# recursiveGecko/Formula-VAD

Measured on AMD Instinct MI355X. Metric: 20ms audio frames/sec end-to-end VAD pipeline, higher is better.
Workload: dtype f32

## Files before the change

formula-vad_amd/binding.py:

```python
import ctypes as C
import os

import numpy as np

_HERE = os.path.dirname(os.path.abspath(__file__))
LIB_PATH = os.environ.get("FVAD_LIB_PATH") or os.path.join(_HERE, "libfvad_hip.so")

c_float_p = C.POINTER(C.c_float)
vp = C.c_void_p
sz = C.c_size_t

FVAD_OK = 0
FVAD_ERR_NO_DEVICE = -101
FVAD_ERR_INVALID_ARGUMENT = -100
FVAD_ERR_OUT_OF_RANGE = -6
FVAD_ERR_NEGATIVE_FREQUENCY = -7
FVAD_ERR_BUFFER_TOO_SMALL = -106
FVAD_ERR_MODEL_FORMAT = -104


class FvadError(RuntimeError):
    def __init__(self, status, where, detail=""):
        self.status = status
        name = lib().fvad_status_name(status).decode()
# ... 808 lines not shown
        try:
            self.close()
        except Exception:
            pass


class VadBatch:

    def __init__(self, n_streams, n_channels=1, sample_rate=48000, fft_size=1024, overrides=None):
        cfg = VadConfig()
        lib().fvad_vad_config_default(C.byref(cfg))
        for k, v in (overrides or {}).items():
            setattr(cfg, k, v)
        self.h = vp()
        check(lib().fvad_vad_batch_create(C.byref(cfg), sample_rate, n_channels, fft_size, n_streams, C.byref(self.h)),
              "fvad_vad_batch_create")
        self.n_streams, self.n_channels = n_streams, n_channels

    def run(self, band, chunk_rms, n_threads=1, chunk_size=24000):
        assert band.dtype == np.float32 and chunk_rms.dtype == np.float32 and band.flags["C_CONTIGUOUS"] and chunk_rms.flags["C_CONTIGUOUS"]
        assert band.shape[0] == chunk_rms.shape[0] == self.n_streams * self.n_channels
        check(lib().fvad_vad_batch_run(self.h, fptr(band), band.shape[1], band.shape[1], fptr(chunk_rms), chunk_rms.shape[1],
                                       chunk_rms.shape[1], chunk_size, n_threads), "fvad_vad_batch_run")
        n = lib().fvad_vad_batch_total_segments(self.h)
        arr = (SpeechSegment * max(n, 1))()
        offs = (sz * (self.n_streams + 1))()
        check(lib().fvad_vad_batch_segments(self.h, arr, max(n, 1), offs), "fvad_vad_batch_segments")
        flat = [(a.sample_from, a.sample_to, a.avg_channel_vol_ratio, a.vad_met_sec) for a in arr[:n]]
        return [flat[offs[s]:offs[s + 1]] for s in range(self.n_streams)]

    def _segments(self):
        n = lib().fvad_vad_batch_total_segments(self.h)
        arr = (SpeechSegment * max(n, 1))()
        offs = (sz * (self.n_streams + 1))()
        check(lib().fvad_vad_batch_segments(self.h, arr, max(n, 1), offs), "fvad_vad_batch_segments")
        flat = [(a.sample_from, a.sample_to, a.avg_channel_vol_ratio, a.vad_met_sec) for a in arr[:n]]
        return [flat[offs[s]:offs[s + 1]] for s in range(self.n_streams)]

    def run_part(self, band, chunk_rms, first_frame, n_threads=1, chunk_size=24000, want_segments=True):
        assert band.dtype == np.float32 and chunk_rms.dtype == np.float32
        assert (band.shape[1] <= 1 or band.strides[1] == 4) and (chunk_rms.shape[1] <= 1 or chunk_rms.strides[1] == 4)
        assert band.shape[0] == chunk_rms.shape[0] == self.n_streams * self.n_channels
        bp = C.cast(band.ctypes.data, c_float_p)
        rp = C.cast(chunk_rms.ctypes.data, c_float_p)
        check(lib().fvad_vad_batch_run_part(self.h, bp, band.strides[0] // 4, band.shape[1], rp, chunk_rms.strides[0] // 4, chunk_rms.shape[1],
                                            chunk_size, first_frame, n_threads), "fvad_vad_batch_run_part")
        return self._segments() if want_segments else None

    def audit(self, stream):
        a = VadAudit()
        check(lib().fvad_vad_batch_audit(self.h, stream, C.byref(a)), "fvad_vad_batch_audit")
        return a.min_rel_threshold_margin, a.min_abs_ratio_margin, a.n_frames

    def close(self):
        if self.h:
            lib().fvad_vad_batch_destroy(self.h)
            self.h = vp()


def _config_array(configs):
    arr = (VadConfig * len(configs))()
    for i, ov in enumerate(configs):
        lib().fvad_vad_config_default(C.byref(arr[i]))
        for k, v in (ov or {}).items():
            setattr(arr[i], k, v)
    return arr


class VadSweep:

    def __init__(self, n_streams, configs, n_channels=1, sample_rate=48000, fft_size=1024):
        self.h = vp()
        check(lib().fvad_vad_batch_create_sweep(_config_array(configs), len(configs), sample_rate, n_channels, fft_size, n_streams,
                                                C.byref(self.h)), "fvad_vad_batch_create_sweep")
        self._created(n_streams, n_channels, len(configs))

    def _created(self, n_streams, n_channels, n_configs):
        self.n_streams, self.n_channels, self.n_configs = n_streams, n_channels, n_configs
        assert lib().fvad_vad_batch_n_configs(self.h) == self.n_configs
        self.sizes, self.size_of_band = self.frame_sizes()

    def frame_sizes(self):
        n = sz()
        sizes = (sz * self.n_configs)()
        sob = (C.c_uint32 * self.n_configs)()
        check(lib().fvad_vad_batch_frame_sizes(self.h, sizes, self.n_configs, C.byref(n), sob), "fvad_vad_batch_frame_sizes")
        n_bands = sz()
        lib().fvad_vad_batch_bands(self.h, None, 0, C.byref(n_bands), None)
        return [sizes[g] for g in range(n.value)], [sob[j] for j in range(n_bands.value)]

    def bands(self):
        n = sz()
        cap = 2 * self.n_configs
        bins = (C.c_int32 * cap)()
        band_of = (C.c_uint32 * self.n_configs)()
        check(lib().fvad_vad_batch_bands(self.h, bins, self.n_configs, C.byref(n), band_of), "fvad_vad_batch_bands")
        return [(bins[2 * j], bins[2 * j + 1]) for j in range(n.value)], list(band_of)

    def size_blocks(self):
        bins, _ = VadSweep.bands(self)
        out = []
        for g, F in enumerate(self.sizes):
            js = [j for j in range(len(bins)) if self.size_of_band[j] == g]
            out.append((F, js[0], [bins[j] for j in js]))
        return out

# ... 423 lines not shown
```

formula-vad_amd/csrc/host_vad.cpp:

```cpp
#include <algorithm>
#include <atomic>
#include <cmath>
#include <cstdlib>
#include <cstring>
#include <memory>
#include <thread>
#include <vector>

#include "host_vad.h"
#include "vad_avgs.h"
#include "vad_finish.h"
#include "vad_ratio.h"

namespace fvad {

RollingAverage::RollingAverage(size_t count, bool has_initial, double initial_val)
    : data(count ? count : 1, 0.0), len(count)
{
    if (has_initial) {
        std::fill(data.begin(), data.begin() + (long)count, initial_val);
        written_count = count;
        avg();
        if (count) enter_steady();
    }
}

double RollingAverage::avg()
{
    double a = 0.0;
    const double scalar = 1.0 / (double)written_count;
    const double* d = data.data();
    for (size_t i = 0; i < written_count; ++i) a += d[i] * scalar;
    last_avg = a;
    has_last_avg = true;
    return a;
}

double RollingAverage::push(float sample)
{
    if (steady) {
        const size_t w = write_idx;
        data[w] = (double)sample;
        q[w] = data[w] * scalar;
        double acc = (w == 0) ? 0.0 : pref;
        acc += q[w];
        const double new_pref = acc;
        const double* qq = q.data();
        for (size_t i = w + 1; i < len; ++i) acc += qq[i];
        last_avg = acc;
        has_last_avg = true;
        write_idx = (w + 1) % len;
        pref = (write_idx == 0) ? 0.0 : new_pref;
        return acc;
    }
    data[write_idx] = (double)sample;
    write_idx = (write_idx + 1) % len;
    if (written_count < len) written_count += 1;
    const double a = avg();
    if (written_count == len && write_idx == 0) enter_steady();
    return a;
}

void RollingAverage::enter_steady()
{
    scalar = 1.0 / (double)len;
    q.resize(len);
    for (size_t i = 0; i < len; ++i) q[i] = data[i] * scalar;
    pref = 0.0;
    for (size_t i = 0; i < write_idx; ++i) pref += q[i];
    steady = true;
}

void Metadata::push(const MetaResult& v, float weight)
{
    if (v.has_ratio) {
        if (!has_ratio) { has_ratio = true; ratio_sum = 0.0f; ratio_weight = 0.0f; }
        ratio_sum += v.volume_ratio * weight;
        ratio_weight += weight;
    }
    if (v.has_min && (!has_min || v.volume_min < volume_min)) { has_min = true; volume_min = v.volume_min; }
    if (v.has_max && (!has_max || v.volume_max > volume_max)) { has_max = true; volume_max = v.volume_max; }
}

MetaResult Metadata::to_result() const
{
    MetaResult r;
    r.has_min = has_min; r.volume_min = volume_min;
    r.has_max = has_max; r.volume_max = volume_max;
    if (has_ratio) { r.has_ratio = true; r.volume_ratio = ratio_sum / ratio_weight; }
    return r;
}

MetaResult analyse_volume(const float* channel_rms, size_t n_channels)
{
    float vol_min = 1, vol_max = 0;
    for (size_t c = 0; c < n_channels; ++c) {
        const float vol = channel_rms[c];
        if (vol < vol_min) vol_min = vol;
        if (vol > vol_max) vol_max = vol;
    }
    MetaResult r;
    r.has_ratio = r.has_min = r.has_max = true;
    r.volume_ratio = (vol_max == 0) ? 0 : vol_min / vol_max;
    r.volume_min = vol_min;
    r.volume_max = vol_max;
    return r;
}

int vad_machine_cfg(const fvad_vad_config& c, size_t sample_rate, size_t fft_size, VadMachineCfg* out)
{
    const float sample_rate_f = (float)sample_rate;
    const float fft_size_f = (float)fft_size;
    const float eval_per_sec = sample_rate_f / fft_size_f;
    const size_t long_len = std::max<size_t>(1, (size_t)(eval_per_sec * c.long_term_speech_avg_sec));
    const size_t short_len = std::max<size_t>(1, (size_t)(eval_per_sec * c.short_term_speech_avg_sec));
    const size_t ratio_len = (size_t)(eval_per_sec * c.channel_vol_ratio_avg_sec);
    VadMachineCfg& k = *out;
    k.lt_scalar = 1.0 / (double)long_len;
    k.st_scalar = 1.0 / (double)short_len;
    k.cr_scalar = 1.0 / (double)ratio_len;
    k.lt_q_init = c.initial_long_term_avg * k.lt_scalar;
    k.initial = c.initial_long_term_avg;
    k.factor = (double)c.speech_threshold_factor;
    k.ratio_threshold = (double)c.channel_vol_ratio_threshold;
    const double n = (double)long_len;
    k.gamma = n * kU / (1.0 - n * kU);
    k.min_open = (uint64_t)(sample_rate_f * c.min_consecutive_sec_to_open);
    k.max_gap = (uint64_t)(sample_rate_f * c.max_speech_gap_sec);
    k.start_buffer = (uint64_t)(sample_rate_f * 2);
    k.end_buffer = (uint64_t)(sample_rate_f * 2);
    k.input_len_sec = fft_size_f / sample_rate_f;
    k.sample_rate_f = sample_rate_f;
    k.min_vad_duration_sec = c.min_vad_duration_sec;
    k.long_len = (uint32_t)long_len;
    k.short_len = (uint32_t)short_len;
    k.ratio_len = (uint32_t)ratio_len;
    k.has_init = c.has_initial_long_term_avg != 0;
    k.band = 0;
    if (ratio_len == 0 || long_len > 0xFFFFFFFFu || short_len > 0xFFFFFFFFu || ratio_len > 0xFFFFFFFFu) return FVAD_ERR_INVALID_ARGUMENT;
    return FVAD_OK;
}

VadMachine::VadMachine(const fvad_vad_config& c, size_t sample_rate, size_t n_channels_, size_t fft_size)
    : n_channels(n_channels_), long_term(1, false, 0), short_term(1, false, 0), ch_ratio(1, false, 0)
{
    vad_machine_cfg(c, sample_rate, fft_size, &cf);
    long_term = RollingAverage(cf.long_len, cf.has_init != 0, cf.initial);
    short_term = RollingAverage(cf.short_len, false, 0);
    ch_ratio = RollingAverage(cf.ratio_len, false, 0);
    lt_last = long_term.last_avg;
    has_last = long_term.has_last_avg;
    segments.reserve(100);
    const char* eager = getenv("FVAD_VAD_EAGER");
    lt_lazy = !(eager && eager[0] == '1');
}

void VadMachine::long_term_exact()
{
    const double* qq = long_term.q.data();
    double acc = 0.0, abs_sum = 0.0;
    for (size_t i = 0; i < long_term.len; ++i) {
        acc += qq[i];
        abs_sum += std::fabs(qq[i]);
    }
    anchor(acc, abs_sum);
}

void VadMachine::long_term_push(float mv)
{
    RollingAverage& a = long_term;
    if (!a.steady || !lt_lazy) {
        const bool was_steady = a.steady;
        lt_last = a.push(mv);
        has_last = true;
        if (lt_lazy && !was_steady && a.steady) long_term_exact();
        return;
    }
    if (!lt_anchored) long_term_exact();
    const size_t w = a.write_idx;
    const double qn = (double)mv * a.scalar, qo = a.q[w];
    a.data[w] = (double)mv;
    a.q[w] = qn;
    a.write_idx = (w + 1) % a.len;
    if (lazy_update(qn, qo)) long_term_exact();
}

float VadMachine::min_volume(const float* channel_volumes) const
{
    float min_v = 999, max_v = 0;
    for (size_t c = 0; c < n_channels; ++c) {
        const float v = channel_volumes[c];
        if (v < min_v) min_v = v;
        if (v > max_v) max_v = v;
    }
    (void)max_v;
    return min_v;
}

fvad_vad_result VadMachine::run(uint64_t index, const float* channel_volumes, bool has_ratio, float ratio)
{
    const float mv = min_volume(channel_volumes);
    const double st = short_term.push(mv);
    const double cr = ch_ratio.push(has_ratio ? ratio : 0);
    const bool met = decide(cf, st, cr, [&] { long_term_exact(); });
    if (!met) long_term_push(mv);
    return finish_step(cf, index, met, has_ratio, ratio, [&](const fvad_speech_segment& s) { segments.push_back(s); });
}

void deal(size_t n, int n_threads, const std::function<void(size_t)>& fn)
{
    const int nt = (int)std::min<size_t>((size_t)std::max(n_threads, 1), n);
    if (nt <= 1) { for (size_t i = 0; i < n; ++i) fn(i); return; }
    std::vector<std::thread> th;
    std::atomic<size_t> next{0};
    for (int t = 0; t < nt; ++t)
        th.emplace_back([&]() { for (;;) { const size_t i = next.fetch_add(1); if (i >= n) break; fn(i); } });
    for (auto& t : th) t.join();
}

void run_many(VadMachine* const* vads, size_t n_streams, const float* const* band,
              const float* const* ratio, const size_t* n_frames, size_t n_channels,
              const uint64_t* first_index, size_t fft_size, int n_threads)
{
    deal(n_streams, n_threads, [&](size_t s) {
        VadMachine* m = vads[s];
        for (size_t k = 0; k < n_frames[s]; ++k) {
            const float r = ratio[s][k];
            const bool has_ratio = !std::isnan(r);
            m->run(first_index[s] + (uint64_t)k * fft_size, band[s] + k * n_channels, has_ratio, r);
        }
    });
}

}

struct fvad_vad { fvad::VadMachine m; fvad_vad(const fvad_vad_config& c, size_t sr, size_t nc, size_t fs) : m(c, sr, nc, fs) {} };
struct fvad_rolling_average { fvad::RollingAverage ra; fvad_rolling_average(size_t n, bool h, double v) : ra(n, h, v) {} };

extern "C" {

void fvad_vad_config_default(fvad_vad_config* c)
{
    c->speech_min_freq = 500; c->speech_max_freq = 2000;
    c->long_term_speech_avg_sec = 180; c->has_initial_long_term_avg = 1; c->initial_long_term_avg = 0.005;
    c->short_term_speech_avg_sec = 0.2f; c->speech_threshold_factor = 10;
    c->channel_vol_ratio_avg_sec = 0.5f; c->channel_vol_ratio_threshold = 0.5f;
    c->min_consecutive_sec_to_open = 0.2f; c->max_speech_gap_sec = 2; c->min_vad_duration_sec = 0.7f;
}

int fvad_vad_create(const fvad_vad_config* cfg, size_t sample_rate, size_t n_channels, size_t fft_size, fvad_vad** out)
{
    if (!cfg || !out || n_channels == 0 || fft_size == 0 || sample_rate == 0) return FVAD_ERR_INVALID_ARGUMENT;
    fvad::VadMachineCfg k;
    if (const int rc = fvad::vad_machine_cfg(*cfg, sample_rate, fft_size, &k)) return rc;
    *out = new (std::nothrow) fvad_vad(*cfg, sample_rate, n_channels, fft_size);
    return *out ? FVAD_OK : FVAD_ERR_ALLOC_FAILED;
}
void fvad_vad_destroy(fvad_vad* v) { delete v; }

int fvad_vad_run(fvad_vad* v, uint64_t index, const float* channel_volumes, int has_ratio, float volume_ratio, fvad_vad_result* out)
{
    if (!v || !channel_volumes) return FVAD_ERR_INVALID_ARGUMENT;
    const fvad_vad_result r = v->m.run(index, channel_volumes, has_ratio != 0, volume_ratio);
    if (out) *out = r;
    return FVAD_OK;
}
size_t fvad_vad_segment_count(const fvad_vad* v) { return v ? v->m.segments.size() : 0; }
int fvad_vad_segments(const fvad_vad* v, fvad_speech_segment* out, size_t cap, size_t* n)
{
    if (!v || !n) return FVAD_ERR_INVALID_ARGUMENT;
    *n = v->m.segments.size();
    if (cap < *n) return FVAD_ERR_BUFFER_TOO_SMALL;
    if (*n) memcpy(out, v->m.segments.data(), *n * sizeof(fvad_speech_segment));
    return FVAD_OK;
}
int fvad_vad_lazy_stats(const fvad_vad* v, uint64_t* exact_evaluations, uint64_t* lazy_pushes)
{
    if (!v) return FVAD_ERR_INVALID_ARGUMENT;
    if (exact_evaluations) *exact_evaluations = v->m.exact_evals;
    if (lazy_pushes) *lazy_pushes = v->m.lazy_pushes;
    return FVAD_OK;
}

int fvad_vad_audit_get(const fvad_vad* v, fvad_vad_audit* out)
{
    if (!v || !out) return FVAD_ERR_INVALID_ARGUMENT;
    *out = v->m.audit;
    return FVAD_OK;
}

int fvad_vad_run_many(fvad_vad* const* vads, size_t n_streams, const float* const* band, const float* const* ratio,
                      const size_t* n_frames, size_t n_channels, const uint64_t* first_index, size_t fft_size, int n_threads)
{
    if (!vads || !band || !ratio || !n_frames || !first_index) return FVAD_ERR_INVALID_ARGUMENT;
    std::vector<fvad::VadMachine*> ms(n_streams);
    for (size_t i = 0; i < n_streams; ++i) {
        if (!vads[i] || vads[i]->m.n_channels != n_channels) return FVAD_ERR_CHANNEL_COUNT_MISMATCH;
        ms[i] = &vads[i]->m;
    }
    fvad::run_many(ms.data(), n_streams, band, ratio, n_frames, n_channels, first_index, fft_size, n_threads);
    return FVAD_OK;
}

int fvad_ra_create(size_t count, int has_initial, double initial_val, fvad_rolling_average** out)
{
    if (!out || count == 0) return FVAD_ERR_INVALID_ARGUMENT;
    *out = new (std::nothrow) fvad_rolling_average(count, has_initial != 0, initial_val);
    return *out ? FVAD_OK : FVAD_ERR_ALLOC_FAILED;
}
void fvad_ra_destroy(fvad_rolling_average* ra) { delete ra; }
double fvad_ra_push(fvad_rolling_average* ra, float sample) { return ra->ra.push(sample); }
int fvad_ra_last_avg(const fvad_rolling_average* ra, double* out)
{
    if (ra->ra.has_last_avg && out) *out = ra->ra.last_avg;
    return ra->ra.has_last_avg ? 1 : 0;
}

int fvad_vad_batch_create(const fvad_vad_config* cfg, size_t sample_rate, size_t n_channels, size_t fft_size, size_t n_streams,
                          fvad_vad_batch** out)
{
    if (!cfg || !out || n_channels == 0 || fft_size == 0 || sample_rate == 0 || n_streams == 0) return FVAD_ERR_INVALID_ARGUMENT;
    fvad::VadMachineCfg k;
    if (const int rc = fvad::vad_machine_cfg(*cfg, sample_rate, fft_size, &k)) return rc;
    auto* b = new (std::nothrow) fvad_vad_batch();
    if (!b) return FVAD_ERR_ALLOC_FAILED;
    b->cfgs.assign(1, *cfg); b->sample_rate = sample_rate; b->n_channels = n_channels; b->fft_size = fft_size; b->n_streams = n_streams;
    const float bin_width = (float)sample_rate / (float)fft_size;
    b->bins = {(int32_t)roundf(cfg->speech_min_freq / bin_width), (int32_t)roundf(cfg->speech_max_freq / bin_width)};
    b->band_of.assign(1, 0);
    b->sizes.assign(1, fft_size); b->size_of.assign(1, 0); b->size_of_band.assign(1, 0);
    b->segs.resize(n_streams);
    b->audits.resize(n_streams);
    b->exact_evals.assign(n_streams, 0);
    b->lazy_pushes.assign(n_streams, 0);
    if (const int rc = fvad::derive_avg_keys(b)) { delete b; return rc; }
    if (const int rc = fvad::derive_trigger_keys(b)) { delete b; return rc; }
    *out = b;
    return FVAD_OK;
}

static int check_sweep_config(const fvad_vad_config& c, size_t sample_rate, size_t fft_size, int32_t* lo, int32_t* hi)
{
    const float bin_width = (float)sample_rate / (float)fft_size;
    const float nyq = (float)sample_rate / 2;
    if (c.speech_min_freq > nyq || c.speech_max_freq > nyq) return FVAD_ERR_OUT_OF_RANGE;
    if (c.speech_min_freq < 0 || c.speech_max_freq < 0) return FVAD_ERR_NEGATIVE_FREQUENCY;
    *lo = (int32_t)roundf(c.speech_min_freq / bin_width);
    *hi = (int32_t)roundf(c.speech_max_freq / bin_width);
    if (*hi < *lo) return FVAD_ERR_INVALID_ARGUMENT;
    fvad::VadMachineCfg k;
    return fvad::vad_machine_cfg(c, sample_rate, fft_size, &k);
}

static int make_sweep(const fvad_vad_config* cfgs, size_t n_configs, const std::vector<size_t>& sizes, const std::vector<uint32_t>& size_of,
                      size_t sample_rate, size_t n_channels, size_t n_streams, fvad_vad_batch** out)
{
    std::vector<std::vector<int32_t>> bins(sizes.size());
    std::vector<uint32_t> local(n_configs);
    for (size_t c = 0; c < n_configs; ++c) {
        int32_t lo = 0, hi = 0;
        const int rc = check_sweep_config(cfgs[c], sample_rate, sizes[size_of[c]], &lo, &hi);
        if (rc) return rc;
        std::vector<int32_t>& bg = bins[size_of[c]];
        size_t j = 0;
        while (j < bg.size() / 2 && !(bg[2 * j] == lo && bg[2 * j + 1] == hi)) ++j;
        if (j == bg.size() / 2) { bg.push_back(lo); bg.push_back(hi); }
        local[c] = (uint32_t)j;
    }
    auto* b = new (std::nothrow) fvad_vad_batch();
    if (!b) return FVAD_ERR_ALLOC_FAILED;
    std::vector<uint32_t> first(sizes.size());
    for (size_t g = 0; g < sizes.size(); ++g) {
        first[g] = (uint32_t)(b->bins.size() / 2);
        b->bins.insert(b->bins.end(), bins[g].begin(), bins[g].end());
        b->size_of_band.insert(b->size_of_band.end(), bins[g].size() / 2, (uint32_t)g);
    }
    b->band_of.resize(n_configs);
    for (size_t c = 0; c < n_configs; ++c) b->band_of[c] = first[size_of[c]] + local[c];
    b->cfgs.assign(cfgs, cfgs + n_configs); b->sample_rate = sample_rate; b->n_channels = n_channels; b->fft_size = sizes[0];
    b->n_streams = n_streams;
    b->sizes = sizes;
    b->size_of = size_of;
    b->segs.resize(n_streams * n_configs);
    b->audits.resize(n_streams * n_configs);
    b->exact_evals.assign(n_streams * n_configs, 0);
    b->lazy_pushes.assign(n_streams * n_configs, 0);
    if (const int rc = fvad::derive_avg_keys(b)) { delete b; return rc; }
    if (const int rc = fvad::derive_trigger_keys(b)) { delete b; return rc; }
    *out = b;
    return FVAD_OK;
}

int fvad_vad_batch_create_sweep(const fvad_vad_config* cfgs, size_t n_configs, size_t sample_rate, size_t n_channels, size_t fft_size,
                                size_t n_streams, fvad_vad_batch** out)
{
    if (!cfgs || !out || n_configs == 0 || n_channels == 0 || fft_size == 0 || sample_rate == 0 || n_streams == 0) return FVAD_ERR_INVALID_ARGUMENT;
    return make_sweep(cfgs, n_configs, {fft_size}, std::vector<uint32_t>(n_configs, 0), sample_rate, n_channels, n_streams, out);
}

int fvad_vad_batch_create_sweep_sized(const fvad_vad_config* cfgs, const size_t* fft_sizes, size_t n_configs, size_t sample_rate,
                                      size_t n_channels, size_t n_streams, fvad_vad_batch** out)
{
    if (!cfgs || !fft_sizes || !out || n_configs == 0 || n_channels == 0 || sample_rate == 0 || n_streams == 0) return FVAD_ERR_INVALID_ARGUMENT;
    std::vector<size_t> sizes;
    std::vector<uint32_t> size_of(n_configs);
    for (size_t c = 0; c < n_configs; ++c) {
        const size_t F = fft_sizes[c];
        if (F < 4 || F > 16384 || F % 2) return FVAD_ERR_INVALID_ARGUMENT;
        size_t g = 0;
        while (g < sizes.size() && sizes[g] != F) ++g;
        if (g == sizes.size()) sizes.push_back(F);
        size_of[c] = (uint32_t)g;
    }
    return make_sweep(cfgs, n_configs, sizes, size_of, sample_rate, n_channels, n_streams, out);
}

int fvad_vad_batch_frame_sizes(const fvad_vad_batch* b, size_t* sizes, size_t cap, size_t* n_sizes, uint32_t* size_of_band)
{
    if (!b || !n_sizes) return FVAD_ERR_INVALID_ARGUMENT;
    *n_sizes = b->sizes.size();
    if (size_of_band) memcpy(size_of_band, b->size_of_band.data(), b->size_of_band.size() * sizeof(uint32_t));
    if (cap < *n_sizes) return FVAD_ERR_BUFFER_TOO_SMALL;
    if (!sizes) return FVAD_ERR_INVALID_ARGUMENT;
    memcpy(sizes, b->sizes.data(), b->sizes.size() * sizeof(size_t));
    return FVAD_OK;
}

void fvad_vad_batch_destroy(fvad_vad_batch* b) { delete b; }

size_t fvad_vad_batch_n_configs(const fvad_vad_batch* b) { return b ? b->cfgs.size() : 0; }

int fvad_vad_batch_avg_keys(const fvad_vad_batch* b, uint32_t* st_keys, uint32_t* cr_keys, size_t cap, size_t* n_st_keys,
                            size_t* n_cr_keys, uint32_t* st_key, uint32_t* cr_key)
{
    if (!b || !n_st_keys || !n_cr_keys) return FVAD_ERR_INVALID_ARGUMENT;
    *n_st_keys = b->st_keys.size() / 2;
    *n_cr_keys = b->cr_keys.size() / 2;
    if (st_key) memcpy(st_key, b->st_key.data(), b->st_key.size() * sizeof(uint32_t));
    if (cr_key) memcpy(cr_key, b->cr_key.data(), b->cr_key.size() * sizeof(uint32_t));
    if (cap < *n_st_keys || cap < *n_cr_keys) return FVAD_ERR_BUFFER_TOO_SMALL;
    if (!st_keys || !cr_keys) return FVAD_ERR_INVALID_ARGUMENT;
// ... 74 lines not shown

namespace fvad {

int derive_avg_keys(fvad_vad_batch* b)
{
    const size_t NC = b->cfgs.size();
    b->st_keys.clear(); b->cr_keys.clear();
    b->st_key.assign(NC, 0); b->cr_key.assign(NC, 0);
    auto find = [](std::vector<uint32_t>& keys, uint32_t src, uint32_t len) {
        size_t j = 0;
        while (j < keys.size() / 2 && !(keys[2 * j] == src && keys[2 * j + 1] == len)) ++j;
        if (j == keys.size() / 2) { keys.push_back(src); keys.push_back(len); }
        return (uint32_t)j;
    };
    for (size_t c = 0; c < NC; ++c) {
        VadMachineCfg k;
        if (const int rc = vad_machine_cfg(b->cfgs[c], b->sample_rate, b->sizes[b->size_of[c]], &k)) return rc;
        b->st_key[c] = find(b->st_keys, b->band_of[c], k.short_len);
        b->cr_key[c] = find(b->cr_keys, b->size_of[c], k.ratio_len);
    }
    return FVAD_OK;
}

int derive_trigger_keys(fvad_vad_batch* b)
{
    struct Key {
        uint32_t size, band, long_len, short_len, ratio_len;
        int32_t has_init;
        uint64_t initial, factor, ratio_threshold;
        bool operator==(const Key& o) const
        {
            return size == o.size && band == o.band && long_len == o.long_len && short_len == o.short_len && ratio_len == o.ratio_len &&
                   has_init == o.has_init && initial == o.initial && factor == o.factor && ratio_threshold == o.ratio_threshold;
        }
    };
    auto bits = [](double d) { uint64_t u; memcpy(&u, &d, 8); return u; };
    const size_t NC = b->cfgs.size();
    std::vector<Key> keys;
    b->trig_key.assign(NC, 0);
    b->trig_rep.clear();
    for (size_t c = 0; c < NC; ++c) {
        VadMachineCfg k;
        if (const int rc = vad_machine_cfg(b->cfgs[c], b->sample_rate, b->sizes[b->size_of[c]], &k)) return rc;
        const Key key{b->size_of[c], b->band_of[c], k.long_len, k.short_len, k.ratio_len, k.has_init, bits(k.initial), bits(k.factor),
                      bits(k.ratio_threshold)};
        size_t j = 0;
        while (j < keys.size() && !(keys[j] == key)) ++j;
        if (j == keys.size()) { keys.push_back(key); b->trig_rep.push_back((uint32_t)c); }
        b->trig_key[c] = (uint32_t)j;
    }
    return FVAD_OK;
}

int retain_stage(const fvad_vad_batch* b, const uint32_t* keep, size_t n_keep, fvad_vad_batch* nb)
{
    const size_t NC = b->cfgs.size(), S = b->n_streams;
    if (n_keep == 0 || !keep) return FVAD_ERR_INVALID_ARGUMENT;
    for (size_t i = 0; i < n_keep; ++i)
        if (keep[i] >= NC || (i && keep[i] <= keep[i - 1])) return FVAD_ERR_INVALID_ARGUMENT;
    try {
        std::vector<uint32_t> size_of(n_keep);
        for (size_t c = 0; c < n_keep; ++c) {
            const size_t F = b->sizes[b->size_of[keep[c]]];
            size_t g = 0;
            while (g < nb->sizes.size() && nb->sizes[g] != F) ++g;
            if (g == nb->sizes.size()) nb->sizes.push_back(F);
            size_of[c] = (uint32_t)g;
        }
        const size_t G = nb->sizes.size();
        std::vector<std::vector<int32_t>> bins(G);
        std::vector<uint32_t> local(n_keep);
        for (size_t c = 0; c < n_keep; ++c) {
            const uint32_t ob = b->band_of[keep[c]];
            const int32_t lo = b->bins[2 * ob], hi = b->bins[2 * ob + 1];
            std::vector<int32_t>& bg = bins[size_of[c]];
            size_t j = 0;
            while (j < bg.size() / 2 && !(bg[2 * j] == lo && bg[2 * j + 1] == hi)) ++j;
            if (j == bg.size() / 2) { bg.push_back(lo); bg.push_back(hi); }
            local[c] = (uint32_t)j;
        }
        std::vector<uint32_t> first(G);
        for (size_t g = 0; g < G; ++g) {
            first[g] = (uint32_t)(nb->bins.size() / 2);
            nb->bins.insert(nb->bins.end(), bins[g].begin(), bins[g].end());
            nb->size_of_band.insert(nb->size_of_band.end(), bins[g].size() / 2, (uint32_t)g);
        }
        nb->band_of.resize(n_keep);
        for (size_t c = 0; c < n_keep; ++c) nb->band_of[c] = first[size_of[c]] + local[c];
        nb->size_of = std::move(size_of);
        nb->sample_rate = b->sample_rate; nb->n_channels = b->n_channels; nb->fft_size = nb->sizes[0]; nb->n_streams = S;
        nb->cfgs.resize(n_keep);
        for (size_t c = 0; c < n_keep; ++c) nb->cfgs[c] = b->cfgs[keep[c]];
        if (const int rc = derive_avg_keys(nb)) return rc;
        if (const int rc = derive_trigger_keys(nb)) return rc;
        const size_t M = S * n_keep;
        nb->segs.resize(M);
        nb->audits.resize(M);
        nb->exact_evals.resize(M);
        nb->lazy_pushes.resize(M);
        if (b->scored) nb->scores.resize(M);
        for (size_t s = 0; s < S; ++s)
            for (size_t c = 0; c < n_keep; ++c) {
                const size_t m = s * n_keep + c, o = s * NC + keep[c];
                nb->audits[m] = b->audits[o];
                nb->exact_evals[m] = b->exact_evals[o];
                nb->lazy_pushes[m] = b->lazy_pushes[o];
                if (b->scored) nb->scores[m] = b->scores[o];
            }
        if (!b->machines.empty()) nb->machines.resize(M);
        if (b->has_refs) {
            nb->refs = b->refs;
            nb->ref_pmax = b->ref_pmax;
            nb->ref_off = b->ref_off;
            nb->stat_cfgs.resize(n_keep);
            for (size_t c = 0; c < n_keep; ++c) nb->stat_cfgs[c] = b->stat_cfgs[keep[c]];
        }
    } catch (const std::bad_alloc&) {
        return FVAD_ERR_ALLOC_FAILED;
    }
    nb->has_refs = b->has_refs;
    nb->scored = b->scored;
    nb->keep_segments = b->keep_segments;
    nb->segs_kept = b->segs_kept;
    nb->next_sample = b->next_sample;
    nb->chain_form = b->chain_form;
    nb->avgs_form = b->avgs_form;
    nb->avgs_bytes = b->avgs_bytes;
    nb->trigger_form = b->trigger_form;
    nb->trigger_bytes = b->trigger_bytes;
    nb->trig_machine_launches = b->trig_machine_launches;
    nb->trig_finish_launches = b->trig_finish_launches;
    return FVAD_OK;
}

void retain_commit(fvad_vad_batch* b, const uint32_t* keep, size_t n_keep, fvad_vad_batch* nb)
{
    const size_t NC = b->cfgs.size();
    for (size_t s = 0; s < b->n_streams; ++s)
        for (size_t c = 0; c < n_keep; ++c) {
            nb->segs[s * n_keep + c] = std::move(b->segs[s * NC + keep[c]]);
            if (!nb->machines.empty()) nb->machines[s * n_keep + c] = std::move(b->machines[s * NC + keep[c]]);
        }
    if (!nb->dev_parts) nb->dev_parts = std::move(b->dev_parts);
    *b = std::move(*nb);
}

}
// ... 10 lines not shown
        out[f] = frame_volume_ratio([&](uint64_t k) { return ratio[(size_t)(k - first_chunk)]; }, (first_frame + f) * fft_size, fft_size, chunk_size);
        if (has) has[f] = 1;
    }
}

void sweep_frame_ratios(const float* chunk_rms, size_t rms_stride, size_t C, size_t n_chunks, size_t n_frames, size_t fft_size,
                        size_t chunk_size, float* out, uint64_t first_frame)
{
    frame_ratios([&](size_t c, size_t k) { return chunk_rms[c * rms_stride + k]; }, C, n_chunks, n_frames, first_frame,
                 first_frame * fft_size / chunk_size, fft_size, chunk_size, out, nullptr);
}

}

extern "C" {

int fvad_vad_batch_frame_ratios(const fvad_vad_batch* b, const float* chunk_rms, size_t rms_stride, const size_t* n_frames,
                                const size_t* n_chunks, size_t chunk_size, uint64_t first_sample, float* ratio, size_t ratio_stride)
{
    if (!b || !n_frames || !n_chunks || chunk_size == 0) return FVAD_ERR_INVALID_ARGUMENT;
    if (first_sample % chunk_size) return FVAD_ERR_INVALID_ARGUMENT;
    const size_t S = b->n_streams, C = b->n_channels, G = b->sizes.size();
    for (size_t g = 0; g < G; ++g) {
        if (first_sample % b->sizes[g]) return FVAD_ERR_INVALID_ARGUMENT;
        for (size_t s = 0; s < S; ++s) {
            const size_t nf = n_frames[g * S + s];
            if (nf > (n_chunks[s] * chunk_size) / b->sizes[g] || nf > ratio_stride || n_chunks[s] > rms_stride) return FVAD_ERR_INVALID_ARGUMENT;
            if (nf && (!chunk_rms || !ratio)) return FVAD_ERR_INVALID_ARGUMENT;
        }
    }
    for (size_t i = 0; i < G * S; ++i) {
        const size_t s = i % S, F = b->sizes[i / S];
        fvad::sweep_frame_ratios(chunk_rms + s * C * rms_stride, rms_stride, C, n_chunks[s], n_frames[i], F, chunk_size, ratio + i * ratio_stride,
                                 first_sample / F);
    }
    return FVAD_OK;
}

}

static int run_host(fvad_vad_batch* b, const float* band, size_t band_stride, const size_t* n_frames, const float* chunk_rms,
                    size_t rms_stride, size_t n_chunks, size_t chunk_size, uint64_t first_sample, int n_threads)
{
    const size_t NC = b->cfgs.size(), G = b->sizes.size();
    if (b->part_in_flight) return FVAD_ERR_INVALID_ARGUMENT;
    if (first_sample != 0 && (first_sample != b->next_sample || b->machines.size() != b->n_streams * NC)) return FVAD_ERR_INVALID_ARGUMENT;
    if (first_sample % chunk_size) return FVAD_ERR_INVALID_ARGUMENT;
    for (size_t g = 0; g < G; ++g) {
        if (first_sample % b->sizes[g]) return FVAD_ERR_INVALID_ARGUMENT;
        if (n_frames[g] * b->sizes[g] > n_chunks * chunk_size) return FVAD_ERR_INVALID_ARGUMENT;
    }
    const uint64_t first_chunk = first_sample / chunk_size;
    const size_t C = b->n_channels, n_lanes = b->n_streams * C;
    if (first_sample == 0) {
        b->dev_parts.reset();
        b->machines.clear();
        for (size_t s = 0; s < b->n_streams; ++s)
            for (size_t c = 0; c < NC; ++c)
                b->machines.emplace_back(new fvad::VadMachine(b->cfgs[c], b->sample_rate, C, b->sizes[b->size_of[c]]));
    }
    auto run_machine = [&](size_t s, size_t c, const float* ratio, const uint8_t* has) {
        fvad::VadMachine& m = *b->machines[s * NC + c];
        const size_t F = b->sizes[b->size_of[c]], nf = n_frames[b->size_of[c]];
        const uint64_t first_frame = first_sample / F;
        const float* bb = band + ((size_t)b->band_of[c] * n_lanes + s * C) * band_stride;
        std::vector<float> vols(C);
        for (size_t f = 0; f < nf; ++f) {
            for (size_t ch = 0; ch < C; ++ch) vols[ch] = bb[ch * band_stride + f];
            m.run((first_frame + f) * F, vols.data(), has[f] != 0, ratio[f]);
        }
        b->segs[s * NC + c] = m.segments;
        b->audits[s * NC + c] = m.audit;
        b->exact_evals[s * NC + c] = m.exact_evals;
        b->lazy_pushes[s * NC + c] = m.lazy_pushes;
    };
    auto stream_ratios = [&](size_t g, size_t s, float* out, uint8_t* has) {
        const size_t F = b->sizes[g];
        fvad::frame_ratios([&](size_t c, size_t k) { return chunk_rms[(s * C + c) * rms_stride + k]; }, C, n_chunks, n_frames[g],
                           first_sample / F, first_chunk, F, chunk_size, out, has);
    };
    if (NC == 1) {
        fvad::deal(b->n_streams, n_threads, [&](size_t s) {
            std::vector<float> ratio(n_frames[0]);
            std::vector<uint8_t> has(n_frames[0]);
            stream_ratios(0, s, ratio.data(), has.data());
            run_machine(s, 0, ratio.data(), has.data());
        });
    } else {
        size_t rs = 0;
        for (size_t g = 0; g < G; ++g) rs = std::max(rs, n_frames[g]);
        const size_t S = b->n_streams;
        std::vector<float> ratio(G * S * rs);
        std::vector<uint8_t> has(G * S * rs);
        fvad::deal(G * S, n_threads, [&](size_t i) { stream_ratios(i / S, i % S, ratio.data() + i * rs, has.data() + i * rs); });
        fvad::deal(S * NC, n_threads, [&](size_t i) {
            const size_t row = ((size_t)b->size_of[i % NC] * S + i / NC) * rs;
            run_machine(i / NC, i % NC, ratio.data() + row, has.data() + row);
        });
    }
    b->next_sample = first_sample + n_frames[0] * b->sizes[0];
    for (size_t g = 1; g < G; ++g)
        if (first_sample + n_frames[g] * b->sizes[g] != b->next_sample) b->next_sample = UINT64_MAX;
    b->segs_kept = true;
    b->scored = false;
    return FVAD_OK;
}

extern "C" {

int fvad_vad_batch_run_part(fvad_vad_batch* b, const float* band, size_t band_stride, size_t n_frames, const float* chunk_rms,
                            size_t rms_stride, size_t n_chunks, size_t chunk_size, uint64_t first_frame, int n_threads)
{
    if (!b || (n_frames && !band) || (n_chunks && !chunk_rms) || chunk_size == 0) return FVAD_ERR_INVALID_ARGUMENT;
    if (b->sizes.size() != 1) return FVAD_ERR_INVALID_ARGUMENT;
    if (first_frame > UINT64_MAX / b->fft_size) return FVAD_ERR_INVALID_ARGUMENT;
// ... 70 lines not shown
```

formula-vad_amd/csrc/host_vad.h:

```cpp
#pragma once
#include <cstddef>
#include <cstdint>
#include <functional>
#include <memory>
#include <vector>

#include "../../include/fvad.h"
#include "vad_machine.h"

namespace fvad {

struct RollingAverage {
    std::vector<double> data;
    size_t len = 0;
    bool has_last_avg = false;
    double last_avg = 0;
    size_t write_idx = 0;
    size_t written_count = 0;
    bool steady = false;
    double scalar = 0, pref = 0;
    std::vector<double> q;
    RollingAverage(size_t count, bool has_initial, double initial_val);
    double push(float sample);
    double avg();
    void enter_steady();
};

struct MetaResult {
    bool has_ratio = false, has_min = false, has_max = false;
    float volume_ratio = 0, volume_min = 0, volume_max = 0;
};
struct Metadata {
    bool has_ratio = false, has_min = false, has_max = false;
    float ratio_sum = 0, ratio_weight = 0, volume_min = 0, volume_max = 0;
    void push(const MetaResult& v, float weight);
    MetaResult to_result() const;
    void reset() { *this = Metadata(); }
};
MetaResult analyse_volume(const float* channel_rms, size_t n_channels);

struct VadMachine : VadMachineState {
    VadMachineCfg cf;
    size_t n_channels;
    RollingAverage long_term, short_term, ch_ratio;
    std::vector<fvad_speech_segment> segments;
    bool lt_lazy = true;
    void long_term_push(float mv);
    void long_term_exact();

    VadMachine(const fvad_vad_config& c, size_t sample_rate, size_t n_channels, size_t fft_size);
    fvad_vad_result run(uint64_t index, const float* channel_volumes, bool has_ratio, float ratio);
    float min_volume(const float* channel_volumes) const;
};

int vad_machine_cfg(const fvad_vad_config& c, size_t sample_rate, size_t fft_size, VadMachineCfg* out);

void deal(size_t n, int n_threads, const std::function<void(size_t)>& fn);

void run_many(VadMachine* const* vads, size_t n_streams, const float* const* band,
              const float* const* ratio, const size_t* n_frames, size_t n_channels,
              const uint64_t* first_index, size_t fft_size, int n_threads);

void sweep_frame_ratios(const float* chunk_rms, size_t rms_stride, size_t n_channels, size_t n_chunks, size_t n_frames, size_t fft_size,
                        size_t chunk_size, float* out, uint64_t first_frame = 0);

struct DevPartsDeleter {
    void (*fn)(void*) = nullptr;
    void operator()(void* p) const { if (fn) fn(p); }
};

}

struct fvad_vad_batch;
namespace fvad {
int derive_avg_keys(fvad_vad_batch* b);
int derive_trigger_keys(fvad_vad_batch* b);
int retain_stage(const fvad_vad_batch* b, const uint32_t* keep, size_t n_keep, fvad_vad_batch* nb);
void retain_commit(fvad_vad_batch* b, const uint32_t* keep, size_t n_keep, fvad_vad_batch* nb);
}

struct fvad_vad_batch {
    std::vector<fvad_vad_config> cfgs;
    std::vector<int32_t> bins;
    std::vector<uint32_t> band_of;
    size_t sample_rate, n_channels, fft_size, n_streams;
    std::vector<size_t> sizes;
    std::vector<uint32_t> size_of, size_of_band;
    std::vector<std::vector<fvad_speech_segment>> segs;
    std::vector<fvad_vad_audit> audits;
    std::vector<uint64_t> exact_evals, lazy_pushes;
    std::vector<std::unique_ptr<fvad::VadMachine>> machines;
    uint64_t next_sample = 0;
    std::unique_ptr<void, fvad::DevPartsDeleter> dev_parts;
    bool part_in_flight = false;
    int chain_form = 0;
    std::vector<uint32_t> st_keys, cr_keys, st_key, cr_key;
    int avgs_form = 0;
    size_t avgs_bytes = 0;
    std::vector<uint32_t> trig_key, trig_rep;
    std::unique_ptr<fvad_vad_batch> trig;
    std::vector<uint32_t> trig_of;
    int trigger_form = 0;
    size_t trigger_bytes = 0;
    uint64_t trig_machine_launches = 0, trig_finish_launches = 0;
    bool has_refs = false;
    std::vector<fvad_segment_sec> refs;
    std::vector<float> ref_pmax;
    std::vector<size_t> ref_off;
    std::vector<fvad_stat_config> stat_cfgs;
    bool scored = false;
    std::vector<fvad_single_stats> scores;
    bool keep_segments = true, segs_kept = true;
};
```

Baseline: 25.54 million.

## Reuse VAD machines, lazily initialize long-term rings, and pool deal threads

Result: no change. 25.59 million, median of 6 (+0.2%).

```diff
diff --git a/formula-vad_amd/binding.py b/formula-vad_amd/binding.py
--- a/formula-vad_amd/binding.py
+++ b/formula-vad_amd/binding.py
@@ -884,6 +884,11 @@
         check(lib().fvad_vad_batch_audit(self.h, stream, C.byref(a)), "fvad_vad_batch_audit")
         return a.min_rel_threshold_margin, a.min_abs_ratio_margin, a.n_frames
 
+    def lazy_stats(self, stream):
+        e, p = C.c_uint64(), C.c_uint64()
+        check(lib().fvad_vad_batch_lazy_stats(self.h, stream, 0, C.byref(e), C.byref(p)), "fvad_vad_batch_lazy_stats")
+        return e.value, p.value
+
     def close(self):
         if self.h:
             lib().fvad_vad_batch_destroy(self.h)
diff --git a/formula-vad_amd/csrc/host_vad.cpp b/formula-vad_amd/csrc/host_vad.cpp
--- a/formula-vad_amd/csrc/host_vad.cpp
+++ b/formula-vad_amd/csrc/host_vad.cpp
@@ -3,8 +3,11 @@
 #include <cmath>
 #include <cstdlib>
 #include <cstring>
+#include <condition_variable>
 #include <memory>
+#include <mutex>
 #include <thread>
+#include <unistd.h>
 #include <vector>
 
 #include "host_vad.h"
@@ -14,22 +17,74 @@
 
 namespace fvad {
 
-RollingAverage::RollingAverage(size_t count, bool has_initial, double initial_val)
-    : data(count ? count : 1, 0.0), len(count)
-{
+void RollingAverage::size_to(size_t count)
+{
+    const size_t n = count ? count : 1;
+    if (n != cap) {
+        data.reset(new double[n]);
+        q.reset(new double[n]);
+        cap = n;
+    }
+    len = count;
+    has_last_avg = false; last_avg = 0;
+    write_idx = 0; written_count = 0;
+    steady = false; scalar = 0; pref = 0;
+    mark = count; init_val = 0; init_q = 0;
+}
+
+void RollingAverage::reset(size_t count, bool has_initial, double initial_val, bool poison)
+{
+    size_to(count);
+    std::fill(data.get(), data.get() + cap, 0.0);
+    if (poison) std::fill(q.get(), q.get() + cap, std::nan(""));
     if (has_initial) {
-        std::fill(data.begin(), data.begin() + (long)count, initial_val);
+        std::fill(data.get(), data.get() + count, initial_val);
         written_count = count;
         avg();
         if (count) enter_steady();
     }
 }
 
+void RollingAverage::reset_pristine(size_t count, double initial_val, const PristineRing& pr, bool poison)
+{
+    size_to(count);
+    if (poison) {
+        std::fill(data.get(), data.get() + cap, std::nan(""));
+        std::fill(q.get(), q.get() + cap, std::nan(""));
+    }
+    written_count = count;
+    last_avg = pr.avg;
+    has_last_avg = true;
+    scalar = 1.0 / (double)count;
+    steady = true;
+    mark = 0;
+    init_val = initial_val;
+    init_q = initial_val * scalar;
+}
+
+PristineRing pristine_ring(size_t len, double initial_val)
+{
+    PristineRing pr;
+    const double scalar = 1.0 / (double)len;
+    double a = 0.0;
+    for (size_t i = 0; i < len; ++i) a += initial_val * scalar;
+    pr.avg = a;
+    const double qi = initial_val * scalar;
+    double acc = 0.0, abs_sum = 0.0;
+    for (size_t i = 0; i < len; ++i) {
+        acc += qi;
+        abs_sum += std::fabs(qi);
+    }
+    pr.acc = acc;
+    pr.abs_sum = abs_sum;
+    return pr;
+}
+
 double RollingAverage::avg()
 {
     double a = 0.0;
     const double scalar = 1.0 / (double)written_count;
-    const double* d = data.data();
+    const double* d = data.get();
     for (size_t i = 0; i < written_count; ++i) a += d[i] * scalar;
     last_avg = a;
     has_last_avg = true;
@@ -45,7 +100,7 @@
         double acc = (w == 0) ? 0.0 : pref;
         acc += q[w];
         const double new_pref = acc;
-        const double* qq = q.data();
+        const double* qq = q.get();
         for (size_t i = w + 1; i < len; ++i) acc += qq[i];
         last_avg = acc;
         has_last_avg = true;
@@ -64,7 +119,6 @@
 void RollingAverage::enter_steady()
 {
     scalar = 1.0 / (double)len;
-    q.resize(len);
     for (size_t i = 0; i < len; ++i) q[i] = data[i] * scalar;
     pref = 0.0;
     for (size_t i = 0; i < write_idx; ++i) pref += q[i];
@@ -141,27 +195,61 @@
     return FVAD_OK;
 }
 
-VadMachine::VadMachine(const fvad_vad_config& c, size_t sample_rate, size_t n_channels_, size_t fft_size)
-    : n_channels(n_channels_), long_term(1, false, 0), short_term(1, false, 0), ch_ratio(1, false, 0)
-{
+int vad_env()
+{
+    const char* eager = getenv("FVAD_VAD_EAGER");
+    const char* poison = getenv("FVAD_VAD_POISON");
+    return (eager && eager[0] == '1' ? kVadEager : 0) | (poison && poison[0] == '1' ? kVadPoison : 0);
+}
+
+VadMachine::VadMachine(const fvad_vad_config& c, size_t sample_rate, size_t n_channels_, size_t fft_size, const PristineRing* pr)
+    : VadMachine(c, sample_rate, n_channels_, fft_size, pr, vad_env())
+{
+}
+
+VadMachine::VadMachine(const fvad_vad_config& c, size_t sample_rate, size_t n_channels_, size_t fft_size, const PristineRing* pr, int env)
+{
+    segments.reserve(100);
+    reset(c, sample_rate, n_channels_, fft_size, pr, env);
+}
+
+void VadMachine::reset(const fvad_vad_config& c, size_t sample_rate, size_t n_channels_, size_t fft_size, const PristineRing* pr, int env)
+{
+    static_cast<VadMachineState&>(*this) = VadMachineState();
+    n_channels = n_channels_;
     vad_machine_cfg(c, sample_rate, fft_size, &cf);
-    long_term = RollingAverage(cf.long_len, cf.has_init != 0, cf.initial);
-    short_term = RollingAverage(cf.short_len, false, 0);
-    ch_ratio = RollingAverage(cf.ratio_len, false, 0);
+    lt_lazy = !(env & kVadEager);
+    const bool poison = (env & kVadPoison) != 0;
+    if (cf.has_init && lt_lazy) {
+        pristine = pr ? *pr : pristine_ring(cf.long_len, cf.initial);
+        long_term.reset_pristine(cf.long_len, cf.initial, pristine, poison);
+    } else {
+        long_term.reset(cf.long_len, cf.has_init != 0, cf.initial, poison);
+    }
+    short_term.reset(cf.short_len, false, 0, poison);
+    ch_ratio.reset(cf.ratio_len, false, 0, poison);
     lt_last = long_term.last_avg;
     has_last = long_term.has_last_avg;
-    segments.reserve(100);
-    const char* eager = getenv("FVAD_VAD_EAGER");
-    lt_lazy = !(eager && eager[0] == '1');
+    segments.clear();
 }
 
 void VadMachine::long_term_exact()
 {
-    const double* qq = long_term.q.data();
+    const RollingAverage& a = long_term;
+    if (a.mark == 0 && a.len) {
+        anchor(pristine.acc, pristine.abs_sum);
+        return;
+    }
+    const double* qq = a.q.get();
     double acc = 0.0, abs_sum = 0.0;
-    for (size_t i = 0; i < long_term.len; ++i) {
+    for (size_t i = 0; i < a.mark; ++i) {
         acc += qq[i];
         abs_sum += std::fabs(qq[i]);
+    }
+    const double qi = a.init_q, abs_qi = std::fabs(qi);
+    for (size_t i = a.mark; i < a.len; ++i) {
+        acc += qi;
+        abs_sum += abs_qi;
     }
     anchor(acc, abs_sum);
 }
@@ -178,9 +266,10 @@
     }
     if (!lt_anchored) long_term_exact();
     const size_t w = a.write_idx;
-    const double qn = (double)mv * a.scalar, qo = a.q[w];
+    const double qn = (double)mv * a.scalar, qo = w < a.mark ? a.q[w] : a.init_q;
     a.data[w] = (double)mv;
     a.q[w] = qn;
+    if (w == a.mark) a.mark = w + 1;
     a.write_idx = (w + 1) % a.len;
     if (lazy_update(qn, qo)) long_term_exact();
 }
@@ -207,10 +296,75 @@
     return finish_step(cf, index, met, has_ratio, ratio, [&](const fvad_speech_segment& s) { segments.push_back(s); });
 }
 
+namespace {
+class DealPool {
+public:
+    ~DealPool()
+    {
+        if (pid != getpid()) { for (auto& t : th) t.detach(); return; }
+        { std::lock_guard<std::mutex> lk(mu); stop = true; }
+        cv_work.notify_all();
+        for (auto& t : th) t.join();
+    }
+    bool run(size_t n_items, int nt, const std::function<void(size_t)>& f)
+    {
+        std::unique_lock<std::mutex> job(job_mu, std::try_to_lock);
+        if (!job || (!th.empty() && pid != getpid())) return false;
+        pid = getpid();
+        while ((int)th.size() < nt - 1) th.emplace_back([this] { worker(); });
+        {
+            std::lock_guard<std::mutex> lk(mu);
+            fn = &f; n = n_items; next = 0; seats = nt - 1; ++gen;
+        }
+        cv_work.notify_all();
+        take(f, n_items);
+        std::unique_lock<std::mutex> lk(mu);
+        seats = 0;
+        cv_done.wait(lk, [&] { return busy == 0; });
+        fn = nullptr;
+        return true;
+    }
+
+private:
+    void take(const std::function<void(size_t)>& f, size_t n_items) noexcept
+    {
+        for (;;) { const size_t i = next.fetch_add(1); if (i >= n_items) break; f(i); }
+    }
+    void worker()
+    {
+        uint64_t seen = 0;
+        std::unique_lock<std::mutex> lk(mu);
+        for (;;) {
+            cv_work.wait(lk, [&] { return stop || (gen != seen && seats > 0); });
+            if (stop) return;
+            seen = gen; --seats; ++busy;
+            const std::function<void(size_t)>* f = fn;
+            const size_t n_items = n;
+            lk.unlock();
+            take(*f, n_items);
+            lk.lock();
+            if (--busy == 0) cv_done.notify_one();
+        }
+    }
+    std::mutex job_mu, mu;
+    std::condition_variable cv_work, cv_done;
+    std::vector<std::thread> th;
+    pid_t pid = 0;
+    const std::function<void(size_t)>* fn = nullptr;
+    size_t n = 0;
+    std::atomic<size_t> next{0};
+    uint64_t gen = 0;
+    int seats = 0, busy = 0;
+    bool stop = false;
+};
+}
+
 void deal(size_t n, int n_threads, const std::function<void(size_t)>& fn)
 {
     const int nt = (int)std::min<size_t>((size_t)std::max(n_threads, 1), n);
     if (nt <= 1) { for (size_t i = 0; i < n; ++i) fn(i); return; }
+    static DealPool pool;
+    if (pool.run(n, nt, fn)) return;
     std::vector<std::thread> th;
     std::atomic<size_t> next{0};
     for (int t = 0; t < nt; ++t)
@@ -234,7 +388,10 @@
 
 }
 
-struct fvad_vad { fvad::VadMachine m; fvad_vad(const fvad_vad_config& c, size_t sr, size_t nc, size_t fs) : m(c, sr, nc, fs) {} };
+struct fvad_vad {
+    fvad::VadMachine m;
+    fvad_vad(const fvad_vad_config& c, size_t sr, size_t nc, size_t fs, const fvad::PristineRing* pr) : m(c, sr, nc, fs, pr) {}
+};
 struct fvad_rolling_average { fvad::RollingAverage ra; fvad_rolling_average(size_t n, bool h, double v) : ra(n, h, v) {} };
 
 extern "C" {
@@ -253,7 +410,8 @@
     if (!cfg || !out || n_channels == 0 || fft_size == 0 || sample_rate == 0) return FVAD_ERR_INVALID_ARGUMENT;
     fvad::VadMachineCfg k;
     if (const int rc = fvad::vad_machine_cfg(*cfg, sample_rate, fft_size, &k)) return rc;
-    *out = new (std::nothrow) fvad_vad(*cfg, sample_rate, n_channels, fft_size);
+    const fvad::PristineRing pr = k.has_init ? fvad::pristine_ring(k.long_len, k.initial) : fvad::PristineRing();
+    *out = new (std::nothrow) fvad_vad(*cfg, sample_rate, n_channels, fft_size, k.has_init ? &pr : nullptr);
     return *out ? FVAD_OK : FVAD_ERR_ALLOC_FAILED;
 }
 void fvad_vad_destroy(fvad_vad* v) { delete v; }
@@ -335,6 +493,7 @@
     b->lazy_pushes.assign(n_streams, 0);
     if (const int rc = fvad::derive_avg_keys(b)) { delete b; return rc; }
     if (const int rc = fvad::derive_trigger_keys(b)) { delete b; return rc; }
+    fvad::derive_pristine(b);
     *out = b;
     return FVAD_OK;
 }
@@ -387,6 +546,7 @@
     b->lazy_pushes.assign(n_streams * n_configs, 0);
     if (const int rc = fvad::derive_avg_keys(b)) { delete b; return rc; }
     if (const int rc = fvad::derive_trigger_keys(b)) { delete b; return rc; }
+    fvad::derive_pristine(b);
     *out = b;
     return FVAD_OK;
 }
@@ -567,6 +727,21 @@
     return FVAD_OK;
 }
 
+void derive_pristine(fvad_vad_batch* b)
+{
+    const size_t NC = b->cfgs.size();
+    std::vector<VadMachineCfg> ks(NC);
+    b->pristine.assign(NC, PristineRing());
+    for (size_t c = 0; c < NC; ++c) {
+        VadMachineCfg& k = ks[c];
+        vad_machine_cfg(b->cfgs[c], b->sample_rate, b->sizes[b->size_of[c]], &k);
+        if (!k.has_init) continue;
+        size_t j = 0;
+        while (j < c && !(ks[j].has_init && ks[j].long_len == k.long_len && memcmp(&ks[j].initial, &k.initial, 8) == 0)) ++j;
+        b->pristine[c] = j < c ? b->pristine[j] : pristine_ring(k.long_len, k.initial);
+    }
+}
+
 int retain_stage(const fvad_vad_batch* b, const uint32_t* keep, size_t n_keep, fvad_vad_batch* nb)
 {
     const size_t NC = b->cfgs.size(), S = b->n_streams;
@@ -608,6 +783,12 @@
         for (size_t c = 0; c < n_keep; ++c) nb->cfgs[c] = b->cfgs[keep[c]];
         if (const int rc = derive_avg_keys(nb)) return rc;
         if (const int rc = derive_trigger_keys(nb)) return rc;
+        if (b->pristine.size() == NC) {
+            nb->pristine.resize(n_keep);
+            for (size_t c = 0; c < n_keep; ++c) nb->pristine[c] = b->pristine[keep[c]];
+        } else {
+            derive_pristine(nb);
+        }
         const size_t M = S * n_keep;
         nb->segs.resize(M);
         nb->audits.resize(M);
@@ -724,15 +905,23 @@
     }
     const uint64_t first_chunk = first_sample / chunk_size;
     const size_t C = b->n_channels, n_lanes = b->n_streams * C;
-    if (first_sample == 0) {
+    const size_t n_machines = b->n_streams * NC;
+    const bool fresh = first_sample == 0;
+    int env = 0;
+    if (fresh) {
         b->dev_parts.reset();
-        b->machines.clear();
-        for (size_t s = 0; s < b->n_streams; ++s)
-            for (size_t c = 0; c < NC; ++c)
-                b->machines.emplace_back(new fvad::VadMachine(b->cfgs[c], b->sample_rate, C, b->sizes[b->size_of[c]]));
+        if (b->machines.size() != n_machines) { b->machines.clear(); b->machines.resize(n_machines); }
+        if (b->pristine.size() != NC) fvad::derive_pristine(b);
+        env = fvad::vad_env();
     }
     auto run_machine = [&](size_t s, size_t c, const float* ratio, const uint8_t* has) {
-        fvad::VadMachine& m = *b->machines[s * NC + c];
+        std::unique_ptr<fvad::VadMachine>& mp = b->machines[s * NC + c];
+        if (fresh) {
+            const size_t Fc = b->sizes[b->size_of[c]];
+            if (mp) mp->reset(b->cfgs[c], b->sample_rate, C, Fc, &b->pristine[c], env);
+            else mp.reset(new fvad::VadMachine(b->cfgs[c], b->sample_rate, C, Fc, &b->pristine[c], env));
+        }
+        fvad::VadMachine& m = *mp;
         const size_t F = b->sizes[b->size_of[c]], nf = n_frames[b->size_of[c]];
         const uint64_t first_frame = first_sample / F;
         const float* bb = band + ((size_t)b->band_of[c] * n_lanes + s * C) * band_stride;
diff --git a/formula-vad_amd/csrc/host_vad.h b/formula-vad_amd/csrc/host_vad.h
--- a/formula-vad_amd/csrc/host_vad.h
+++ b/formula-vad_amd/csrc/host_vad.h
@@ -10,8 +10,14 @@
 
 namespace fvad {
 
+struct PristineRing {
+    double avg = 0;
+    double acc = 0, abs_sum = 0;
+};
+
 struct RollingAverage {
-    std::vector<double> data;
+    std::unique_ptr<double[]> data, q;
+    size_t cap = 0;
     size_t len = 0;
     bool has_last_avg = false;
     double last_avg = 0;
@@ -19,12 +25,19 @@
     size_t written_count = 0;
     bool steady = false;
     double scalar = 0, pref = 0;
-    std::vector<double> q;
-    RollingAverage(size_t count, bool has_initial, double initial_val);
+    size_t mark = 0;
+    double init_val = 0, init_q = 0;
+    RollingAverage() = default;
+    RollingAverage(size_t count, bool has_initial, double initial_val) { reset(count, has_initial, initial_val, false); }
+    void reset(size_t count, bool has_initial, double initial_val, bool poison);
+    void reset_pristine(size_t count, double initial_val, const PristineRing& pr, bool poison);
     double push(float sample);
     double avg();
     void enter_steady();
+private:
+    void size_to(size_t count);
 };
+PristineRing pristine_ring(size_t len, double initial_val);
 
 struct MetaResult {
     bool has_ratio = false, has_min = false, has_max = false;
@@ -45,13 +58,19 @@
     RollingAverage long_term, short_term, ch_ratio;
     std::vector<fvad_speech_segment> segments;
     bool lt_lazy = true;
+    PristineRing pristine;
     void long_term_push(float mv);
     void long_term_exact();
 
-    VadMachine(const fvad_vad_config& c, size_t sample_rate, size_t n_channels, size_t fft_size);
+    VadMachine(const fvad_vad_config& c, size_t sample_rate, size_t n_channels, size_t fft_size, const PristineRing* pr = nullptr);
+    VadMachine(const fvad_vad_config& c, size_t sample_rate, size_t n_channels, size_t fft_size, const PristineRing* pr, int env);
+    void reset(const fvad_vad_config& c, size_t sample_rate, size_t n_channels, size_t fft_size, const PristineRing* pr, int env);
     fvad_vad_result run(uint64_t index, const float* channel_volumes, bool has_ratio, float ratio);
     float min_volume(const float* channel_volumes) const;
 };
+
+enum { kVadEager = 1, kVadPoison = 2 };
+int vad_env();
 
 int vad_machine_cfg(const fvad_vad_config& c, size_t sample_rate, size_t fft_size, VadMachineCfg* out);
 
@@ -75,6 +94,7 @@
 namespace fvad {
 int derive_avg_keys(fvad_vad_batch* b);
 int derive_trigger_keys(fvad_vad_batch* b);
+void derive_pristine(fvad_vad_batch* b);
 int retain_stage(const fvad_vad_batch* b, const uint32_t* keep, size_t n_keep, fvad_vad_batch* nb);
 void retain_commit(fvad_vad_batch* b, const uint32_t* keep, size_t n_keep, fvad_vad_batch* nb);
 }
@@ -90,6 +110,7 @@
     std::vector<fvad_vad_audit> audits;
     std::vector<uint64_t> exact_evals, lazy_pushes;
     std::vector<std::unique_ptr<fvad::VadMachine>> machines;
+    std::vector<fvad::PristineRing> pristine;
     uint64_t next_sample = 0;
     std::unique_ptr<void, fvad::DevPartsDeleter> dev_parts;
     bool part_in_flight = false;
```
